# adolliou/euispice_coreg

Hardware: AMD Instinct MI355X
Metric: lag-points/sec (whole node) on 2048² grid, 60×60 CRVAL sweep; argmax-shift match (higher is better)
Workload: dtype f64; 1 GPU; headline: Carrington 'fa' 2048x2048 grid lon(200,300) lat(-20,20), 60x60 CRVAL lags arange(-30,30,1) arcsec, small 2048^2 HRIEUV-like, ref 3072^2 FSI-like, order 2, solar_r 1.004; lag_points=3600, parallelism=single GPU, no collective, resident=True, sweeps_in_flight=2, small_stored_f32=True, use_lds=True

## Files before the change

euispice_coreg_amd/csrc/host_plan.hpp:

```cpp
#pragma once
namespace {

struct ComboRange {
    long long begin = 0, end = 0;
};
ComboRange take_combo_range(coreg_handle* h) {
    ComboRange r;
    r.begin = h->opt_combo_begin;
    r.end = h->opt_combo_end;
    h->opt_combo_begin = h->opt_combo_end = 0;
    return r;
}
int check_lags(coreg_handle* h, const coreg_lags* l, LagDims* d, int64_t begin, int64_t end, ComboRange combo = ComboRange()) {
    if (!l || !l->crval1 || !l->crval2 || !l->cdelt1 || !l->cdelt2 || !l->crota)
        return fail(h, COREG_EINVAL, "lags: null array");
    if (l->n_crval1 < 1 || l->n_crval2 < 1 || l->n_cdelt1 < 1 || l->n_cdelt2 < 1 || l->n_crota < 1)
        return fail(h, COREG_EINVAL, "lags: every axis needs at least one value");
    d->n1 = l->n_crval1;
    d->n2 = l->n_crval2;
    d->n3 = l->n_cdelt1;
    d->n4 = l->n_cdelt2;
    d->n5 = l->n_crota;
    d->nc = (long long)d->n3 * d->n4 * d->n5;
    d->c0 = 0;
// ... 34 lines not shown

long long lds_window_elems(const coreg_handle* h);
SweepEnv sweep_env(coreg_handle* h) {
    SweepEnv e;
    e.sW = h->sW;
    e.sH = h->sH;
    e.gW = h->gW;
    e.gH = h->gH;
    e.border_fix = h->opt_border_fix != 0;
    e.tap_fix = h->opt_tap_fix != 0;
    e.use_lds = h->opt_use_lds != 0;
    e.h_series = h->opt_h_series != 0;
    e.tile_skip = h->opt_tile_skip != 0;
    e.lds_elems = lds_window_elems(h);
    e.tile_w = (int)h->opt_tile_w;
    e.patch_w = (int)h->opt_patch_w;
    e.shard_world = h->opt_shard_world;
    e.n_groups = h->opt_n_groups;
    e.pitch = h->opt_pitch;
    e.tabs = &h->tabs;
    e.caches = &h->wcslib;
    e.memo = &h->plan_memo;
    return e;
}

void pick_taper(const coreg_handle* h, int n_groups, int n_batches, int* tmin, int* tfrac) {
    *tmin = (int)h->opt_taper_min;
    if (h->opt_taper_frac >= 0) {
        *tfrac = (int)h->opt_taper_frac;
        return;
    }
    const double rounds = (double)n_groups * n_batches / 256.0;
    *tfrac = (rounds >= (double)h->opt_taper_rounds && n_groups >= 128 && h->opt_shard_world <= 1) ? 512 : 0;
}

template <int MODE>
int launch_precompute(coreg_handle* h, const PrecomputeArgs& a, int n_tiles, int n_groups, int n_batches) {
    EventPair* ev = next_event(h, h->ev_pre, h->ev_pre_used);
    if (!ev) return fail(h, COREG_EHIP, "hipEventCreate failed");
    int tmin, tfrac;
    pick_taper(h, n_groups, n_batches, &tmin, &tfrac);
    PrecomputeArgs b = a;
    b.prologue = h->pending_prologue;
    const bool with_prologue = b.prologue.src != nullptr;
    std::memset(&h->pending_prologue, 0, sizeof(h->pending_prologue));
    HIPCHK(hipEventRecord(ev->a, h->stream));
    if (h->ref_dtype == COREG_F32)
        hipLaunchKernelGGL((k_precompute<MODE, float>), dim3(n_tiles), dim3(256), 0, h->stream, b);
    else
        hipLaunchKernelGGL((k_precompute<MODE, double>), dim3(n_tiles), dim3(256), 0, h->stream, b);
    (void)with_prologue;
    hipLaunchKernelGGL(k_tile_list, dim3(1), dim3(1024), 0, h->stream, (const int*)a.tile_count, n_tiles, n_groups,
                       h->tile_list.as<int>(), h->tile_cum.as<int>(), h->group_first.as<int>(),
                       h->tile_info.as<long long>(), tmin, tfrac);
    ev->b_is_next_sweep = true;
    ev->next_sweep_index = h->ev_sweep_used;
    HIPCHK(hipGetLastError());
    return COREG_OK;
}

int reserve_tiles(coreg_handle* h, int n_tiles) {
    const size_t pts = (size_t)n_tiles * kTilePts + (size_t)(kPointGroups + 1) * kChunk;
    HIPCHK(h->pts.reserve(pts * sizeof(Pt)));
    HIPCHK(h->tile_count.reserve(n_tiles * sizeof(int)));
    HIPCHK(h->tile_list.reserve(n_tiles * sizeof(int)));
    HIPCHK(h->tile_cum.reserve((n_tiles + 1) * sizeof(int)));
    HIPCHK(h->group_first.reserve(2 * 1024 * sizeof(int) + 64));
    HIPCHK(h->tile_info.reserve(8 * sizeof(long long)));
    HIPCHK(h->tile_bbox.reserve((size_t)n_tiles * 4 * sizeof(double)));
    return COREG_OK;
}

int setup_precompute(coreg_handle* h, const Plan& plan, int method, PrecomputeArgs* a, int* n_tiles) {
    std::memset(a, 0, sizeof(*a));
    a->tile_w = plan.tile_w;
    a->tile_h = kTilePts / plan.tile_w;
    a->tiles_x = (h->gW + a->tile_w - 1) / a->tile_w;
    a->tiles_y = (h->gH + a->tile_h - 1) / a->tile_h;
    *n_tiles = a->tiles_x * a->tiles_y;
    RETCHK(reserve_tiles(h, *n_tiles));
    a->ref = h->ref.p;
    a->gw = h->gW;
    a->gh = h->gH;
    a->pivot_a = h->pivots.as<double>();
    a->pts = h->pts.as<Pt>();
    a->tile_count = h->tile_count.as<int>();
    a->tile_bbox = h->tile_bbox.as<double>();
    a->residus = method != COREG_METHOD_CORRELATION ? 1 : 0;
    return COREG_OK;
}

}
```

euispice_coreg_amd/csrc/host_state.hpp:

```cpp
#pragma once
namespace {

enum SrcKind {
    SRC_HOST = 0,
    SRC_PINNED = 1,
    SRC_DEVICE = 2,
    SRC_TILED = 3,
};

struct PixFmt {
    int bitpix = 0;
    bool f32 = false;
    double bscale = 1.0, bzero = 0.0;
    bool raw() const { return bitpix != 0; }
    bool scaled() const { return bscale != 1.0 || bzero != 0.0; }
    size_t elem() const { return raw() ? (size_t)(bitpix < 0 ? -bitpix : bitpix) / 8 : (f32 ? 4 : 8); }
    bool swap_only() const { return bitpix == -32 && !scaled(); }
    static PixFmt native(bool is_f32) {
        PixFmt f;
        f.f32 = is_f32;
        return f;
    }
};

// ... 5 lines not shown
    bool b_is_next_sweep = false;
    size_t next_sweep_index = 0;
};

}

struct KeptTapLists {
    DevBuf all;
};
struct TapFix {
    TapFixArgs args = {};
    int segs = 0;
    int mode = 0;
    long long count = 0;
};
struct FixLaunch {
    std::vector<BorderFixArgs> border;
    std::vector<ParityFixArgs> parity;
    TapFix tap;
    std::shared_ptr<KeptTapLists> kept;
    bool small_f32 = true;
    bool empty() const { return border.empty() && parity.empty() && tap.segs == 0; }
};

struct ContextState;
struct PixelsState;

struct coreg_handle {
    int device = 0;
    Stream stream;
    std::string err;

    std::unique_ptr<ContextState> ctx;
    std::unique_ptr<PixelsState> pix;
    ~coreg_handle();

    DevBuf small;
    int sW = 0, sH = 0;
    bool small_f32 = false;
    DevBuf ref;
    int gW = 0, gH = 0;
    int ref_dtype = -1;
    DevBuf pivots, red_sum, red_cnt;
    DevBuf t_sin_lon, t_cos_lon, t_cos_lat, t_sin_lat, t_lon_deg, t_dx;
    coreg_diffrot rot_ref = {}, rot_small = {};
    bool has_rot_ref = false, has_rot_small = false;
    CarrTables tabs;
    std::vector<double> tabs_key;
    bool tabs_uploaded = false;
    PinBuf pin_img[2];
    Event ev_img[2];
    int pin_img_next = 0;
    DevBuf pts, tile_count, tile_list, tile_cum, group_first, tile_info, tile_bbox;
    DevBuf rf_fix_slab;
    DevBuf counters;
    DevBuf lane_params, out_index, partials, out_dev, tmp_img;
    DevBuf counts;
    long long counts_n = -1;
    DevBuf up_f64, up_flag;
    DevBuf up_raw;
    DevBuf rice_blob, rice_rand, dec_img;
    PrologueArgs pending_prologue = {};
    DevBuf bbox_buf;
    Stream aux_stream;
    Stream up_stream;
    Event ev_small, ev_main;
    bool small_pending = false;
    DevBuf red_sum_up, red_cnt_up;
    int64_t opt_overlap_upload = 1;
    int64_t opt_tap_nan_filter = 2;
    int64_t opt_async_upload = 0;
    std::thread up_thread;
    std::mutex up_m;
    std::condition_variable up_cv;
    std::function<hipError_t()> up_job;
    bool up_has = false, up_stop = false, up_busy = false;
    hipError_t up_rc = hipSuccess;
    PinBuf pin_small[2];
    Event ev_pin_small[2];
    int pin_small_next = 0;
    WcslibCaches wcslib;
    DevBuf border_flags, fix_partial;
    DevBuf border_dev;
    PinBuf pin_border;
    int64_t opt_border_fix = 1;
    int64_t opt_tap_fix = 1, opt_tap_cap = 1 << 24;
    DevBuf tap_count, tap_segq, tap_list, tap_skip, tap_seg_slot, tap_seg_begin, tap_pixel, tap_xw, tap_yw;
    long long tap_last[3] = {0, 0, 0};
    int last_variant[7] = {-1, 0, 0, 0, 0, 0, 0};
    int64_t opt_shard_world = 1, opt_shard_rank = 0;
    int64_t opt_combo_begin = 0, opt_combo_end = 0;
    DevBuf sums;
    long long sums_slots = 0;
    struct PendingFinalize {
        long long slot_off, n_slots, lag_begin;
        int residus;
        RefineArgs refine;
        std::function<int(coreg_handle*)> replay_precompute;
        FixLaunch fixes;
    };
    std::function<int(coreg_handle*)> last_precompute;
    PlanMemo plan_memo;
    DevBuf rf_flags, rf_pivots, rf_list, rf_head, rf_partial;
    std::vector<PendingFinalize> pending_fin;
    DevBuf fin_outidx;
    long long pending_n_out = 0;
// ... 22 lines not shown
```

euispice_coreg_amd/csrc/host_sweep_launch.hpp:

```cpp
#pragma once
namespace {
using sweep_variant::SweepVariant;
static_assert(sweep_variant::kTranslate == MODE_TRANSLATE && sweep_variant::kHomography == MODE_HOMOGRAPHY &&
                  sweep_variant::kHomographySeries == MODE_HOMOGRAPHY_SERIES && sweep_variant::kCar == MODE_CAR &&
                  sweep_variant::kOrderRt == ORDER_RT, "sweep_variant.hpp restates the kernels' constants");

struct SweepLaunchSpec {
    int mode = MODE_TRANSLATE;
    int order = 2;
    int method = COREG_METHOD_CORRELATION;
    size_t slot_off = 0;
    int n_batches = 0, n_tiles = 0;
    long long lag_begin = 0;
    double* out_dev = nullptr;
    const LaunchU* car_inv = nullptr;
    const BorderFix* fix = nullptr;
    int pitch_sel = 0;
    long long n_slots() const { return (long long)n_batches * kBlock; }
    bool residus() const { return method != COREG_METHOD_CORRELATION; }
    int residus_kind() const { return method == COREG_METHOD_RESIDUS_MASKED ? 2 : (residus() ? 1 : 0); }
    const double* params_dev(const coreg_handle* h) const {
        return h->lane_params.as<double>() + (mode == MODE_TRANSLATE ? 2 : 9) * slot_off;
    }
    const long long* outidx_dev(const coreg_handle* h) const { return h->out_index.as<long long>() + slot_off; }
};

struct SweepKernel {
    void (*fn)(const SweepArgs);
    size_t attr_bytes[kMaxDevices];
};
template <size_t... I>
SweepKernel* sweep_kernel_table(std::index_sequence<I...>) {
    constexpr const SweepVariant* v = sweep_variant::kSweepVariants.v;
    static SweepKernel table[] = {
        {k_sweep<v[I].mode, v[I].order, std::conditional_t<v[I].f32, float, double>, v[I].round, v[I].resid, v[I].pitch>, {0}}...};
    return table;
}

int raise_dynamic_lds(coreg_handle* h, SweepKernel* k, size_t lds_bytes) {
    std::lock_guard<std::mutex> lock(g_attr_mutex);
    size_t& ab = k->attr_bytes[h->device % kMaxDevices];
    if (lds_bytes > 48 * 1024 && lds_bytes > ab) {
        HIPCHK(hipFuncSetAttribute((const void*)k->fn, hipFuncAttributeMaxDynamicSharedMemorySize, (int)lds_bytes));
        ab = lds_bytes;
    }
    return COREG_OK;
}

int launch_k_sweep(coreg_handle* h, const SweepLaunchSpec& L, const SweepArgs& a, dim3 grid, size_t lds_bytes) {
    const SweepVariant v = sweep_variant::pick_sweep_variant(L.mode, L.order, h->small_f32, L.residus(), L.pitch_sel);
    const int at = sweep_variant::sweep_variant_index(v);
    if (at < 0) return fail(h, COREG_EINVAL, "launch_sweep: no k_sweep instantiation for this mode / order / pitch");
    SweepKernel* k = sweep_kernel_table(std::make_index_sequence<sweep_variant::kNumSweepVariants>()) + at;
    EventPair* ev = next_event(h, h->ev_sweep, h->ev_sweep_used);
    if (!ev) return fail(h, COREG_EHIP, "hipEventCreate failed");
    RETCHK(raise_dynamic_lds(h, k, lds_bytes));
    HIPCHK(hipEventRecord(ev->a, h->stream));
    hipLaunchKernelGGL(k->fn, grid, dim3(kSweepThreads), lds_bytes, h->stream, a);
    HIPCHK(hipEventRecord(ev->b, h->stream));
    HIPCHK(hipGetLastError());
    const int rec[7] = {at, v.mode, v.order, v.f32 ? 1 : 0, v.round ? 1 : 0, v.resid ? 1 : 0, v.pitch};
    std::copy(rec, rec + 7, h->last_variant);
    return COREG_OK;
}

SweepArgs sweep_args(const coreg_handle* h, const SweepLaunchSpec& L, int n_groups, int group_lo, size_t lds_bytes) {
    SweepArgs a;
    a.img = h->small.p;
    a.W = h->sW;
    a.H = h->sH;
    a.pts = h->pts.as<Pt>();
    a.tile_count = h->tile_count.as<int>();
    a.tile_list = h->tile_list.as<int>();
    a.tile_cum = h->tile_cum.as<int>();
    a.group_first = h->group_first.as<int>();
    a.tile_info = h->tile_info.as<long long>();
    a.tile_bbox = h->tile_bbox.as<double>();
    a.lane_params = L.params_dev(h);
    a.n_slots = L.n_slots();
    a.n_batches = L.n_batches;
    a.n_groups = n_groups;
    a.group_lo = group_lo;
    a.partials = h->partials.as<double>();
    a.pivots = h->pivots.as<double>();
    a.use_lds = h->opt_use_lds ? 1 : 0;
    a.clean_path = h->opt_clean_path ? 1 : 0;
    a.lds_elems = (int)(lds_bytes / sizeof(double));
    a.car_inv = L.car_inv ? *L.car_inv : LaunchU{};
    a.car_inv.order_rt = L.order;
    a.car_inv.h_incr = (int)h->opt_h_incr;
    return a;
}

template <typename Args>
void fill_fix_common(Args& x, const coreg_handle* h, const SweepLaunchSpec& L) {
    x.img = h->small.p;
    x.W = h->sW;
    x.H = h->sH;
    x.ref = h->ref.p;
    x.ref_f32 = h->ref_dtype == COREG_F32 ? 1 : 0;
    x.gw = h->gW;
    x.order = L.order;
    x.round_f32 = L.mode == MODE_TRANSLATE ? 0 : 1;
    x.residus = L.residus() ? 1 : 0;
    x.pivots = h->pivots.as<double>();
    x.hom = L.params_dev(h);
    x.n_slots = L.n_slots();
}

int build_fix_launch(coreg_handle* h, const SweepLaunchSpec& L, FixLaunch* fl) {
    fl->small_f32 = h->small_f32;
    if (!L.fix || !L.fix->any()) return COREG_OK;
    static const std::vector<BorderItems::Item> no_items;
    for (const BorderItems::Item& it : L.fix->border ? L.fix->border->items : no_items) {
        if (it.flags_off >= 0) {
            ParityFixArgs p = {};
            fill_fix_common(p, h, L);
            p.flags = h->border_flags.as<unsigned char>() + it.flags_off;
            p.gh = h->gH;
            p.slot = it.slot;
            p.n_partial = 256;
            if (h->fix_partial.reserve((size_t)p.n_partial * kNumSums * sizeof(double)) != hipSuccess)
                return fail(h, COREG_EHIP, "hipMalloc failed (parity fix)");
            p.partial = h->fix_partial.as<double>();
            fl->parity.push_back(p);
        }
        if (it.n == 0) continue;
        BorderFixArgs b = {};
        fill_fix_common(b, h, L);
        b.slot = it.slot;
// ... 111 lines not shown
```

euispice_coreg_amd/csrc/kernels_prepare.hpp:

```cpp
#pragma once
namespace coreg {
template <typename T>
__global__ void __launch_bounds__(256) k_sum_finite(const T* __restrict__ v, long long n, double* part_sum,
                                                    long long* part_cnt) {
    __shared__ double ss[256];
    __shared__ long long sc[256];
    double s = 0.0;
    long long c = 0;
    for (long long i = (long long)blockIdx.x * 256 + threadIdx.x; i < n; i += (long long)gridDim.x * 256) {
        const double x = (double)v[i];
        if (isfinite(x)) {
            s += x;
            ++c;
        }
    }
    ss[threadIdx.x] = s;
    sc[threadIdx.x] = c;
    __syncthreads();
    for (int o = 128; o > 0; o >>= 1) {
        if ((int)threadIdx.x < o) {
            ss[threadIdx.x] += ss[threadIdx.x + o];
            sc[threadIdx.x] += sc[threadIdx.x + o];
        }
        __syncthreads();
// ... 262 lines not shown
                pt.pad = st;
            }
            a.pts[tbase + off + rank] = pt;
            mn0 = fmin(mn0, b0);
            mx0 = fmax(mx0, b0);
            mn1 = fmin(mn1, b1);
            mx1 = fmax(mx1, b1);
        }
        base_pos += tot;
        __syncthreads();
    }
    if (MODE != MODE_CAR && !a.residus) {
        static_assert(kChunk >= 3, "run flag + the two chunk sums live in the pads of the chunk's first three points");
        Pt* tp = a.pts + tbase;
        for (int c = threadIdx.x; c < base_pos / kChunk; c += 256) {
            double sa = tp[c * kChunk].a, saa = sa * sa;
            bool run = MODE == MODE_HOMOGRAPHY || MODE == MODE_HOMOGRAPHY_SERIES;
#pragma unroll
            for (int k = 1; k < kChunk; ++k) {
                const double v = tp[c * kChunk + k].a;
                sa += v;
                saa = fma(v, v, saa);
                run = run && tp[c * kChunk + k].b0 == tp[c * kChunk].b0 + (double)k && tp[c * kChunk + k].b1 == tp[c * kChunk].b1;
            }
            tp[c * kChunk].pad = run ? 1.0 : 0.0;
            tp[c * kChunk + 1].pad = sa;
            tp[c * kChunk + 2].pad = saa;
        }
    }
    for (int o = 32; o > 0; o >>= 1) {
        mn0 = fmin(mn0, __shfl_xor(mn0, o));
        mx0 = fmax(mx0, __shfl_xor(mx0, o));
        mn1 = fmin(mn1, __shfl_xor(mn1, o));
        mx1 = fmax(mx1, __shfl_xor(mx1, o));
    }
    if (lane == 0) {
        red[wave][0] = mn0;
        red[wave][1] = mx0;
        red[wave][2] = mn1;
        red[wave][3] = mx1;
    }
    __syncthreads();
    if (threadIdx.x == 0) {
        a.tile_count[tile] = base_pos;
        double* bb = a.tile_bbox + (size_t)tile * 4;
        bb[0] = fmin(fmin(red[0][0], red[1][0]), fmin(red[2][0], red[3][0]));
        bb[1] = fmax(fmax(red[0][1], red[1][1]), fmax(red[2][1], red[3][1]));
        bb[2] = fmin(fmin(red[0][2], red[1][2]), fmin(red[2][2], red[3][2]));
        bb[3] = fmax(fmax(red[0][3], red[1][3]), fmax(red[2][3], red[3][3]));
    }
}

constexpr int kUnitPts = kChunk * kPointGroups;
__host__ __device__ inline long long group_start(int g, long long total, int n_groups, int taper_min, int taper_frac) {
    if (taper_frac <= 0) return (long long)g * total / n_groups;
    const int g0 = n_groups - (int)((long long)n_groups * taper_frac / 1024);
    const int nt = n_groups - 1 - g0;
    if (nt <= 0) return (long long)g * total / n_groups;
    const double m = (double)taper_min / 1024.0;
    auto cum = [&](int k) -> double {
        if (k <= g0) return (double)k;
        const double j = (double)(k - g0);
        return (double)g0 + j - (1.0 - m) * j * (j - 1.0) / (2.0 * (double)nt);
    };
    if (g >= n_groups) return total;
    const long long s0 = (long long)(cum(g) / cum(n_groups) * (double)total);
    return s0 < 0 ? 0 : (s0 > total ? total : s0);
}
__global__ void __launch_bounds__(1024) k_tile_list(const int* __restrict__ tile_count, int n_tiles, int n_groups,
                                                    int* tile_list, int* tile_cum, int* group_first, long long* info,
                                                    int taper_min, int taper_frac) {
    __shared__ int wcnt[16];
    __shared__ int wunits[16];
    __shared__ long long wpts[16];
    __shared__ int s_base, s_units;
    __shared__ long long s_pts;
    const int lane = threadIdx.x & 63, wave = threadIdx.x >> 6;
    if (threadIdx.x == 0) {
        s_base = 0;
        s_units = 0;
        s_pts = 0;
    }
    __syncthreads();
    for (int t0 = 0; t0 < n_tiles; t0 += 1024) {
        const int t = t0 + threadIdx.x;
        const int c = t < n_tiles ? tile_count[t] : 0;
        const bool nz = c > 0;
        const int units = (c + kUnitPts - 1) / kUnitPts;
        const unsigned long long bal = __ballot(nz);
        const int rank = __popcll(bal & ((1ull << lane) - 1ull));
        long long pts = c;
        int uincl = units;
        for (int o = 1; o < 64; o <<= 1) {
            const int v = __shfl_up(uincl, o);
            if (lane >= o) uincl += v;
        }
        for (int o = 32; o > 0; o >>= 1) pts += __shfl_xor(pts, o);
        if (lane == 63) wunits[wave] = uincl;
        if (lane == 0) {
            wcnt[wave] = __popcll(bal);
            wpts[wave] = pts;
        }
        __syncthreads();
        int off = s_base, uoff = s_units;
        for (int w = 0; w < wave; ++w) {
            off += wcnt[w];
            uoff += wunits[w];
        }
        if (nz) {
            tile_list[off + rank] = t;
            tile_cum[off + rank] = uoff + uincl - units;
        }
        __syncthreads();
        if (threadIdx.x == 0) {
            int tot = 0, tu = 0;
            long long tp = 0;
            for (int w = 0; w < 16; ++w) {
                tot += wcnt[w];
                tu += wunits[w];
                tp += wpts[w];
            }
            s_base += tot;
            s_units += tu;
            s_pts += tp;
        }
        __syncthreads();
    }
    const int n_list = s_base, total = s_units;
    if (threadIdx.x == 0) {
        tile_cum[n_list] = total;
        info[0] = n_list;
        info[1] = s_pts;
        info[2] = total;
        info[3] = info[4] = info[5] = info[6] = 0;
    }
    __syncthreads();
    for (int g = threadIdx.x; g <= n_groups; g += 1024) {
        const long long start = group_start(g, total, n_groups, taper_min, taper_frac);
        group_first[1024 + g] = (int)start;
        int lo = 0, hi = n_list;
        while (lo < hi) {
            const int mid = (lo + hi + 1) >> 1;
            if (mid <= n_list && (long long)tile_cum[mid] <= start) lo = mid;
            else hi = mid - 1;
        }
        group_first[g] = lo;
    }
}

}
```

euispice_coreg_amd/csrc/kernels_sweep.hpp:

```cpp
#pragma once
namespace coreg {
struct SweepArgs {
    const void* img;
    int W, H;
    const Pt* pts;
    const int* tile_count;
    const int* tile_list;
    const int* tile_cum;
    const int* group_first;
    long long* tile_info;
    const double* tile_bbox;
    const double* lane_params;
    long long n_slots;
    int n_batches;
    int n_groups;
    int group_lo;
    double* partials;
    const double* pivots;
    int use_lds;
    int clean_path;
    int lds_elems;
    LaunchU car_inv;
};

struct Acc {
    int n;
    double a, b, aa, bb, ab;
};

template <int N>
struct Taps;
template <>
struct Taps<3> {
    double t[9];
    __device__ __forceinline__ void issue(unsigned a0, unsigned a1, unsigned a2) {
        asm volatile(
            "ds_read_b64 %0, %9\n\tds_read_b64 %1, %9 offset:8\n\tds_read_b64 %2, %9 offset:16\n\t"
            "ds_read_b64 %3, %10\n\tds_read_b64 %4, %10 offset:8\n\tds_read_b64 %5, %10 offset:16\n\t"
            "ds_read_b64 %6, %11\n\tds_read_b64 %7, %11 offset:8\n\tds_read_b64 %8, %11 offset:16"
            : "=&v"(t[0]), "=&v"(t[1]), "=&v"(t[2]), "=&v"(t[3]), "=&v"(t[4]), "=&v"(t[5]), "=&v"(t[6]), "=&v"(t[7]),
              "=&v"(t[8])
            : "v"(a0), "v"(a1), "v"(a2));
    }
    __device__ __forceinline__ void wait_after(double& w0, double& w1, double& w2, double& w3, double& w4, double& w5) {
        asm volatile("s_waitcnt lgkmcnt(0)"
                     : "+v"(t[0]), "+v"(t[1]), "+v"(t[2]), "+v"(t[3]), "+v"(t[4]), "+v"(t[5]), "+v"(t[6]), "+v"(t[7]),
                       "+v"(t[8]), "+v"(w0), "+v"(w1), "+v"(w2), "+v"(w3), "+v"(w4), "+v"(w5));
    }
    __device__ __forceinline__ void issue_before(unsigned a0, unsigned a1, unsigned a2, double& fx, double& fy) {
        asm volatile(
            "ds_read_b64 %0, %11\n\tds_read_b64 %1, %11 offset:8\n\tds_read_b64 %2, %11 offset:16\n\t"
            "ds_read_b64 %3, %12\n\tds_read_b64 %4, %12 offset:8\n\tds_read_b64 %5, %12 offset:16\n\t"
            "ds_read_b64 %6, %13\n\tds_read_b64 %7, %13 offset:8\n\tds_read_b64 %8, %13 offset:16"
            : "=&v"(t[0]), "=&v"(t[1]), "=&v"(t[2]), "=&v"(t[3]), "=&v"(t[4]), "=&v"(t[5]), "=&v"(t[6]), "=&v"(t[7]),
              "=&v"(t[8]), "+v"(fx), "+v"(fy)
            : "v"(a0), "v"(a1), "v"(a2));
    }
    __device__ __forceinline__ void wait() {
        asm volatile("s_waitcnt lgkmcnt(0)"
                     : "+v"(t[0]), "+v"(t[1]), "+v"(t[2]), "+v"(t[3]), "+v"(t[4]), "+v"(t[5]), "+v"(t[6]), "+v"(t[7]),
                       "+v"(t[8]));
    }
    template <int P>
    __device__ __forceinline__ void issue_before_imm(unsigned a0, double& fx, double& fy) {
// ... 312 lines not shown
        } else if (isfinite(v)) {
            acc.n += 1;
            acc.a += av;
            acc.b += bm;
            acc.aa = fma(av, av, acc.aa);
            acc.bb = fma(bm, bm, acc.bb);
            acc.ab = fma(av, bm, acc.ab);
        }
    }
}

#ifndef COREG_PT_SCALAR
#define COREG_PT_SCALAR 2
#endif
#ifndef COREG_PT_ANCHOR
#define COREG_PT_ANCHOR 1
#endif
typedef unsigned SPt __attribute__((ext_vector_type(8)));
__device__ __forceinline__ SPt spt_load(const Pt* __restrict__ p, double& anchor) {
    SPt r;
#if defined(__HIP_DEVICE_COMPILE__)
#if COREG_PT_ANCHOR
    asm volatile("s_load_dwordx8 %0, %2, 0x0" : "=s"(r), "+v"(anchor) : "s"(p));
#else
    asm volatile("s_load_dwordx8 %0, %1, 0x0" : "=s"(r) : "s"(p));
#endif
#else
    r = (SPt)(0u);
    (void)p;
    (void)anchor;
#endif
    return r;
}
__device__ __forceinline__ void spt_wait(SPt& r) {
#if defined(__HIP_DEVICE_COMPILE__)
    asm volatile("s_waitcnt lgkmcnt(0)" : "+s"(r));
#endif
}
__device__ __forceinline__ double spt_f64(const SPt& r, int i) {
    const unsigned long long u = ((unsigned long long)r[2 * i + 1] << 32) | (unsigned long long)r[2 * i];
    return __builtin_bit_cast(double, u);
}
__device__ __forceinline__ void load_pt_uniform(const Pt* __restrict__ p, Pt& out) {
#if defined(__HIP_DEVICE_COMPILE__) && COREG_PT_SCALAR
    typedef const __attribute__((address_space(4))) double* ConstF64;
    ConstF64 q = (ConstF64)(const double*)p;
    out.b0 = q[0];
    out.b1 = q[1];
    out.a = q[2];
    out.pad = q[3];
#else
    out = *p;
#endif
}

template <int MODE, int ORDER, typename TS, bool LDS, bool ROUND, bool RESID, bool INTERIOR = false, int PITCH = 0,
          bool CLEAN = false>
__device__ __forceinline__ void tile_points(Acc& acc, unsigned win, const TS* __restrict__ img, int pitch,
                                            int ox, int oy, int W, int H, double px0, double py0, double pxw,
                                            double pyw, const H9& hm, const LaunchU& cu, const Pt* __restrict__ pts, int p_begin, int p_end,
                                            double pivot_b, int pg) {
    const double wmax = (double)(W - 1), hmax = (double)(H - 1);
    const int n_full = p_end / kChunk;
#if defined(__HIP_DEVICE_COMPILE__) && COREG_PT_SCALAR == 2
    constexpr bool kIncr = INTERIOR && LDS && ORDER == 2 && !RESID &&
                           (MODE == MODE_HOMOGRAPHY || MODE == MODE_HOMOGRAPHY_SERIES);
    if constexpr (kIncr) {
        if (cu.h_incr) {
            H9 hv = hm;
            hv.h[0] = fma(pxw, hm.h[6], hm.h[0]);
            hv.h[1] = fma(pxw, hm.h[7], hm.h[1]);
            hv.h[2] = MODE == MODE_HOMOGRAPHY_SERIES ? hm.h[2] + pxw : fma(pxw, hm.h[8], hm.h[2]);
            hv.h[3] = fma(pyw, hm.h[6], hm.h[3]);
            hv.h[4] = fma(pyw, hm.h[7], hm.h[4]);
            hv.h[5] = MODE == MODE_HOMOGRAPHY_SERIES ? hm.h[5] + pyw : fma(pyw, hm.h[8], hm.h[5]);
            int c = p_begin / kChunk + pg;
            if (c < n_full) {
                double& anchor = hv.h[7];
                SPt cur = spt_load(pts + c * kChunk, anchor);
                spt_wait(cur);
                for (; c < n_full; c += kPointGroups) {
                    const Pt* __restrict__ q = pts + c * kChunk;
                    const bool run = cur[7] != 0u;
                    double xn = 0.0, yn = 0.0, ww = 0.0;
#pragma unroll
                    for (int k = 0; k < kChunk; ++k) {
                        SPt nxt = spt_load(k + 1 < kChunk ? q + k + 1 : q + kPointGroups * kChunk, anchor);
                        const double x = spt_f64(cur, 0), y = spt_f64(cur, 1);
                        if (k == 0 || !run) {
                            xn = fma(hv.h[0], x, fma(hv.h[1], y, hv.h[2]));
                            yn = fma(hv.h[3], x, fma(hv.h[4], y, hv.h[5]));
                            ww = MODE == MODE_HOMOGRAPHY_SERIES ? fma(hv.h[6], x, hv.h[7] * y)
                                                                : fma(hv.h[6], x, fma(hv.h[7], y, hv.h[8]));
                        } else {
                            xn += hv.h[0];
                            yn += hv.h[3];
                            ww += hv.h[6];
                        }
                        double ux, uy;
                        if (MODE == MODE_HOMOGRAPHY_SERIES) {
                            const double qq = fma(ww, ww, -ww);
                            ux = fma(xn, qq, xn);
                            uy = fma(yn, qq, yn);
                        } else {
                            double r = __builtin_amdgcn_rcp(ww);
                            r = fma(r, fma(-ww, r, 1.0), r);
// ... 75 lines not shown
            load_pt_uniform(pts + p, pt);
            point_lag<MODE, ORDER, TS, LDS, ROUND, RESID, INTERIOR, PITCH>(acc, win, img, pitch, ox, oy, W, H, wmax, hmax,
                                                                           px0, py0, pxw, pyw, hm, cu, pt.b0, pt.b1, pt.a,
                                                                           pt.pad, pivot_b);
        }
    }
}

template <int MODE, int ORDER, typename TS, bool ROUND, bool RESID, int PITCH = 0>
__global__ void __launch_bounds__(kSweepThreads) k_sweep(const SweepArgs a) {
    extern __shared__ __align__(16) unsigned char lds_raw[];
    double* lds = (double*)lds_raw;
    constexpr int kWaves = kSweepThreads / 64;
    constexpr int kLagWaves = kBlock / 64;
    __shared__ double wred2[2][kLagWaves][4];
    __shared__ int wdirty[2][kWaves];
    constexpr bool kCleanPath = MODE != MODE_CAR && !RESID && ORDER != ORDER_RT && !(ROUND && sizeof(TS) == 8);
    int visit = 0;
    int n_vis = 0, n_vis_lds = 0, n_vis_int = 0, n_vis_clean = 0;

    const int b = blockIdx.x;
    const int slot8 = b & 7;
    const int q = b >> 3;
    const int batch = q % a.n_batches;
    const int group = a.group_lo + (q / a.n_batches) * 8 + slot8;

    const int lane = threadIdx.x & 63, wave = threadIdx.x >> 6;
    const int pg = __builtin_amdgcn_readfirstlane(wave % kPointGroups);
    const int lw = __builtin_amdgcn_readfirstlane(wave / kPointGroups);
    const int ls = 64 * lw + lane;
    const long long slot = (long long)batch * kBlock + ls;

    double px0 = 0.0, py0 = 0.0;
    H9 hm;
#pragma unroll
    for (int k = 0; k < 9; ++k) hm.h[k] = 0.0;
    if (MODE == MODE_TRANSLATE) {
        px0 = a.lane_params[slot];
        py0 = a.lane_params[a.n_slots + slot];
    } else {
#pragma unroll
        for (int k = 0; k < 9; ++k) hm.h[k] = a.lane_params[(long long)k * a.n_slots + slot];
    }

    const bool pad_lane = MODE == MODE_TRANSLATE ? (px0 != px0) : (hm.h[8] != hm.h[8]);

    Acc acc = {0, 0.0, 0.0, 0.0, 0.0, 0.0};

    const TS* __restrict__ img = (const TS*)a.img;
    const int W = a.W, H = a.H;
    const double inf = __builtin_inf();
    const int u_lo = a.group_first[1024 + group];
    const int u_hi = a.group_first[1024 + group + 1];
    const int n_list = (int)a.tile_info[0];
    const double pivot_b = a.pivots[1];
#if defined(__HIP_DEVICE_COMPILE__)
    const unsigned win = (unsigned)(uintptr_t)(__attribute__((address_space(3))) unsigned char*)lds_raw;
#else
    const unsigned win = 0;
#endif

    for (int tl = a.group_first[group]; tl < n_list && u_lo < u_hi; ++tl) {
        const int ubase = a.tile_cum[tl];
        if (ubase >= u_hi) break;
        const int tile = a.tile_list[tl];
        const int cnt = a.tile_count[tile];
        const int p_begin = max(u_lo - ubase, 0) * kUnitPts;
        const int p_end = min((u_hi - ubase) * kUnitPts, cnt);
        if (p_begin >= p_end) continue;
        const double* bb = a.tile_bbox + (size_t)tile * 4;
        const double bx0 = bb[0], bx1 = bb[1], by0 = bb[2], by1 = bb[3];

        double mnx, mxx, mny, mxy;
        if (MODE == MODE_TRANSLATE) {
            mnx = bx0 + px0;
            mxx = bx1 + px0;
            mny = by0 + py0;
            mxy = by1 + py0;
        } else {
            mnx = inf; mxx = -inf; mny = inf; mxy = -inf;
#pragma unroll
            for (int c = 0; c < 4; ++c) {
                double cx, cy;
                apply_map<MODE>(hm, a.car_inv, (c & 1) ? bx1 : bx0, (c & 2) ? by1 : by0, cx, cy);
                mnx = fmin(mnx, cx);
                mxx = fmax(mxx, cx);
                mny = fmin(mny, cy);
                mxy = fmax(mxy, cy);
            }
            if (MODE == MODE_CAR) {
                const double margin = car_tile_margin(a.car_inv.box_c, fmax(fabs(by0), fabs(by1)) + a.car_inv.pole_sep);
                mnx -= margin;
                mxx += margin;
                mny -= margin;
                mxy += margin;
            }
        }
        for (int o = 32; o > 0; o >>= 1) {
            mnx = fmin(mnx, __shfl_xor(mnx, o));
            mxx = fmax(mxx, __shfl_xor(mxx, o));
            mny = fmin(mny, __shfl_xor(mny, o));
            mxy = fmax(mxy, __shfl_xor(mxy, o));
        }
        double(*wred)[4] = wred2[visit & 1];
        int* wdirt = wdirty[visit & 1];
        ++visit;
        if (lane == 0 && pg == 0) {
            wred[lw][0] = mnx;
            wred[lw][1] = mxx;
            wred[lw][2] = mny;
            wred[lw][3] = mxy;
        }
        __syncthreads();
        mnx = fmin(fmin(wred[0][0], wred[1][0]), fmin(wred[2][0], wred[3][0]));
        mxx = fmax(fmax(wred[0][1], wred[1][1]), fmax(wred[2][1], wred[3][1]));
        mny = fmin(fmin(wred[0][2], wred[1][2]), fmin(wred[2][2], wred[3][2]));
        mxy = fmax(fmax(wred[0][3], wred[1][3]), fmax(wred[2][3], wred[3][3]));
        if (!(mxx >= 0.0) || !(mnx <= (double)(W - 1)) || !(mxy >= 0.0) || !(mny <= (double)(H - 1))) continue;
        constexpr double kClear = 1e-9;
        const bool interior = (mnx >= kClear) & (mxx <= (double)(W - 1) - kClear) & (mny >= kClear) &
                              (mxy <= (double)(H - 1) - kClear);
        constexpr bool kWide = ORDER == ORDER_RT || ORDER > 2;
        const int ord = ORDER == ORDER_RT ? a.car_inv.order_rt : ORDER;
        const int ap_lo = kWide ? ord / 2 + 1 : 1;
        const int ap_hi = kWide ? ord - ord / 2 + 1 : 2;
        const int ox = max((int)floor(fmax(mnx, 0.0)) - ap_lo, kWide ? -ap_lo : -1);
        const int oy = max((int)floor(fmax(mny, 0.0)) - ap_lo, kWide ? -ap_lo : -1);
        const int ex = min((int)floor(fmin(mxx, (double)(W - 1))) + ap_hi, kWide ? W - 1 + ap_hi : W);
        const int ey = min((int)floor(fmin(mxy, (double)(H - 1))) + ap_hi, kWide ? H - 1 + ap_hi : H);
        const int ww = ex - ox + 1, wh = ey - oy + 1;
        int pitch = PITCH > 0 ? PITCH : (ww | 1);
        if (PITCH == 0) {
            const int r = pitch & 31;
            const int up = r < 5 ? 5 - r : ((r > 11 && r < 21) ? 21 - r : (r > 27 ? 37 - r : 0));
            if ((long long)(pitch + up) * wh <= (long long)a.lds_elems) pitch += up;
        }
        const long long need = (long long)pitch * wh;
        const bool in_lds = a.use_lds && (need <= (long long)a.lds_elems) && (PITCH == 0 || ww <= PITCH);

        const Pt* __restrict__ pts = a.pts + (size_t)tile * kTilePts;

        bool swept = false;
        ++n_vis;
        {
          if (in_lds) {
            swept = true;
            ++n_vis_lds;
#ifndef COREG_STAGE_ROWS
#define COREG_STAGE_ROWS 8
#endif
#ifndef COREG_STAGE_COLS
#define COREG_STAGE_COLS 1
#endif
            constexpr int kStage = COREG_STAGE_ROWS, kCols = COREG_STAGE_COLS;
            const double scale = ORDER == 2 ? 0.25 : 1.0;
            const int wave_u = __builtin_amdgcn_readfirstlane(wave);
            double poison = 0.0;
            for (int r0 = wave_u; r0 < wh; r0 += kWaves * kStage) {
                for (int c0 = 0; c0 < ww; c0 += 64 * kCols) {
                    int gx[kCols];
#pragma unroll
                    for (int j = 0; j < kCols; ++j) {
                        const int c = c0 + 64 * j + lane;
                        gx[j] = kWide ? mirror_far(ox + min(c, ww - 1), W) : mirror_idx(ox + min(c, ww - 1), W);
                    }
                    TS v[kStage][kCols];
#pragma unroll
                    for (int k = 0; k < kStage; ++k) {
                        const int r = min(r0 + k * kWaves, wh - 1);
                        const int gy = kWide ? mirror_far(oy + r, H) : mirror_idx(oy + r, H);
                        const TS* __restrict__ row = img + (size_t)gy * W;
#pragma unroll
                        for (int j = 0; j < kCols; ++j) v[k][j] = row[gx[j]];
                    }
#pragma unroll
                    for (int j = 0; j < kCols; ++j) {
                        const int c = c0 + 64 * j + lane;
                        if (c < ww) {
#pragma unroll
                            for (int k = 0; k < kStage; ++k) {
                                const int r = r0 + k * kWaves;
                                if (r < wh) {
                                    const double e = (ROUND ? (double)v[k][j] : (double)v[k][j] - pivot_b) * scale;
                                    lds[r * pitch + c] = e;
                                    if (kCleanPath) poison = fma(e, 0.0, poison);
                                }
                            }
                        }
                    }
                }
            }
            if (kCleanPath && interior) {
                const int dirty = __ballot(poison != poison) != 0ull;
                if (lane == 0) wdirt[wave] = dirty;
            }
            __syncthreads();
            bool done = false;
            if constexpr (ORDER != ORDER_RT) {
                if (interior) {
                    done = true;
                    bool clean = false;
                    if constexpr (kCleanPath) clean = a.clean_path && __ballot(wdirt[lane % kWaves] != 0) == 0ull;
                    ++n_vis_int;
                    n_vis_clean += clean ? 1 : 0;
                    if (!pad_lane) {
                        const double offx = (ORDER == 2 ? 0.5 : 0.0) - (double)(ORDER / 2 + ox);
                        const double offy = (ORDER == 2 ? 0.5 : 0.0) - (double)(ORDER / 2 + oy);
                        const double pxw = MODE == MODE_TRANSLATE ? px0 + offx : offx;
                        const double pyw = MODE == MODE_TRANSLATE ? py0 + offy : offy;
                        if (kCleanPath && clean) {
                            tile_points<MODE, ORDER, TS, true, ROUND, RESID, true, PITCH, kCleanPath>(
                                acc, win, img, pitch, ox, oy, W, H, px0, py0, pxw, pyw, hm, a.car_inv, pts, p_begin, p_end,
                                pivot_b, pg);
                        } else {
                            tile_points<MODE, ORDER, TS, true, ROUND, RESID, true, PITCH>(acc, win, img, pitch, ox, oy, W, H,
                                                                                          px0, py0, pxw, pyw, hm, a.car_inv,
                                                                                          pts, p_begin, p_end, pivot_b, pg);
                        }
                    }
                }
            }
            if (!done) {
                const double offx = ORDER == 2 ? 0.5 - (double)(1 + ox) : (ORDER == 3 ? -(double)(1 + ox) : 0.0);
                const double offy = ORDER == 2 ? 0.5 - (double)(1 + oy) : (ORDER == 3 ? -(double)(1 + oy) : 0.0);
                tile_points<MODE, ORDER, TS, true, ROUND, RESID, false, PITCH>(acc, win, img, pitch, ox, oy, W, H, px0, py0,
                                                                               offx, offy, hm, a.car_inv, pts, p_begin,
                                                                               p_end, pivot_b, pg);
            }
          }
        }
        if (!swept) {
            tile_points<MODE, ORDER, TS, false, ROUND, RESID>(acc, win, img, 0, 0, 0, W, H, px0, py0, 0.0, 0.0, hm, a.car_inv, pts,
                                                              p_begin, p_end, pivot_b, pg);
        }
    }

    if (threadIdx.x == 0) {
        atomicAdd((unsigned long long*)a.tile_info + 3, (unsigned long long)n_vis);
        atomicAdd((unsigned long long*)a.tile_info + 4, (unsigned long long)n_vis_lds);
        atomicAdd((unsigned long long*)a.tile_info + 5, (unsigned long long)n_vis_int);
        atomicAdd((unsigned long long*)a.tile_info + 6, (unsigned long long)n_vis_clean);
    }
    __syncthreads();
    if (pg > 0) {
        double* st = lds + ((size_t)(pg - 1) * kNumSums) * kBlock + ls;
        st[0] = (double)acc.n;
        st[kBlock] = acc.a;
        st[2 * kBlock] = acc.b;
        st[3 * kBlock] = acc.aa;
        st[4 * kBlock] = acc.bb;
        st[5 * kBlock] = acc.ab;
    }
    __syncthreads();
    if (pg == 0) {
        double sn = (double)acc.n, sa = acc.a, sb = acc.b, saa = acc.aa, sbb = acc.bb, sab = acc.ab;
        for (int g = 0; g < kPointGroups - 1; ++g) {
            const double* st = lds + ((size_t)g * kNumSums) * kBlock + ls;
            sn += st[0];
            sa += st[kBlock];
            sb += st[2 * kBlock];
            saa += st[3 * kBlock];
            sbb += st[4 * kBlock];
            sab += st[5 * kBlock];
        }
        double* out = a.partials + (size_t)(group - a.group_lo) * kNumSums * a.n_slots + slot;
        out[0] = sn;
        out[a.n_slots] = sa;
        out[2 * a.n_slots] = sb;
        out[3 * a.n_slots] = saa;
        out[4 * a.n_slots] = sbb;
        out[5 * a.n_slots] = sab;
    }
}

}
```

Baseline: 1.208 million lag-points/s.

## Pack per-visit tile records, prefetch next visit, hoist lag bounding box

Builds a 64-byte VisitRec per listed tile (cumulative units, tile id, count, bbox) in k_tile_list. The sweep kernel loads each record through scalar constant-address loads, prefetches the next one and parks it in a VGPR via writelane. For translate mode it computes the lag bounding box once per block, so the per-visit wave shuffle reduction and one barrier per visit go away. It also folds the order-2 staging subtract-and-scale into a single FMA. The intent is to cut dependent global loads and syncs per tile visit, at the cost of a looser (union-over-lanes) window bound and more staged rows.

```diff
diff --git a/euispice_coreg_amd/csrc/host_plan.hpp b/euispice_coreg_amd/csrc/host_plan.hpp
--- a/euispice_coreg_amd/csrc/host_plan.hpp
+++ b/euispice_coreg_amd/csrc/host_plan.hpp
@@ -110,7 +110,8 @@
     (void)with_prologue;
     hipLaunchKernelGGL(k_tile_list, dim3(1), dim3(1024), 0, h->stream, (const int*)a.tile_count, n_tiles, n_groups,
                        h->tile_list.as<int>(), h->tile_cum.as<int>(), h->group_first.as<int>(),
-                       h->tile_info.as<long long>(), tmin, tfrac);
+                       h->tile_info.as<long long>(), tmin, tfrac, (const double*)a.tile_bbox,
+                       h->visit_rec.as<VisitRec>());
     ev->b_is_next_sweep = true;
     ev->next_sweep_index = h->ev_sweep_used;
     HIPCHK(hipGetLastError());
@@ -126,6 +127,7 @@
     HIPCHK(h->group_first.reserve(2 * 1024 * sizeof(int) + 64));
     HIPCHK(h->tile_info.reserve(8 * sizeof(long long)));
     HIPCHK(h->tile_bbox.reserve((size_t)n_tiles * 4 * sizeof(double)));
+    HIPCHK(h->visit_rec.reserve(((size_t)n_tiles + 1) * sizeof(VisitRec)));
     return COREG_OK;
 }
 
diff --git a/euispice_coreg_amd/csrc/host_state.hpp b/euispice_coreg_amd/csrc/host_state.hpp
--- a/euispice_coreg_amd/csrc/host_state.hpp
+++ b/euispice_coreg_amd/csrc/host_state.hpp
@@ -81,6 +81,7 @@
     Event ev_img[2];
     int pin_img_next = 0;
     DevBuf pts, tile_count, tile_list, tile_cum, group_first, tile_info, tile_bbox;
+    DevBuf visit_rec;
     DevBuf rf_fix_slab;
     DevBuf counters;
     DevBuf lane_params, out_index, partials, out_dev, tmp_img;
diff --git a/euispice_coreg_amd/csrc/host_sweep_launch.hpp b/euispice_coreg_amd/csrc/host_sweep_launch.hpp
--- a/euispice_coreg_amd/csrc/host_sweep_launch.hpp
+++ b/euispice_coreg_amd/csrc/host_sweep_launch.hpp
@@ -76,6 +76,7 @@
     a.group_first = h->group_first.as<int>();
     a.tile_info = h->tile_info.as<long long>();
     a.tile_bbox = h->tile_bbox.as<double>();
+    a.visit_rec = h->visit_rec.as<VisitRec>();
     a.lane_params = L.params_dev(h);
     a.n_slots = L.n_slots();
     a.n_batches = L.n_batches;
diff --git a/euispice_coreg_amd/csrc/kernels_prepare.hpp b/euispice_coreg_amd/csrc/kernels_prepare.hpp
--- a/euispice_coreg_amd/csrc/kernels_prepare.hpp
+++ b/euispice_coreg_amd/csrc/kernels_prepare.hpp
@@ -338,6 +338,12 @@
 }
 
 constexpr int kUnitPts = kChunk * kPointGroups;
+struct alignas(64) VisitRec {
+    int tile_cum, tile, count, pad;
+    double bbox[4];
+    double fill[2];
+};
+static_assert(sizeof(VisitRec) == 64, "one record per 64-byte line");
 __host__ __device__ inline long long group_start(int g, long long total, int n_groups, int taper_min, int taper_frac) {
     if (taper_frac <= 0) return (long long)g * total / n_groups;
     const int g0 = n_groups - (int)((long long)n_groups * taper_frac / 1024);
@@ -355,7 +361,8 @@
 }
 __global__ void __launch_bounds__(1024) k_tile_list(const int* __restrict__ tile_count, int n_tiles, int n_groups,
                                                     int* tile_list, int* tile_cum, int* group_first, long long* info,
-                                                    int taper_min, int taper_frac) {
+                                                    int taper_min, int taper_frac,
+                                                    const double* __restrict__ tile_bbox, VisitRec* visit_rec) {
     __shared__ int wcnt[16];
     __shared__ int wunits[16];
     __shared__ long long wpts[16];
@@ -396,6 +403,15 @@
         if (nz) {
             tile_list[off + rank] = t;
             tile_cum[off + rank] = uoff + uincl - units;
+            VisitRec r;
+            r.tile_cum = uoff + uincl - units;
+            r.tile = t;
+            r.count = c;
+            r.pad = 0;
+#pragma unroll
+            for (int k = 0; k < 4; ++k) r.bbox[k] = tile_bbox[(size_t)t * 4 + k];
+            r.fill[0] = r.fill[1] = 0.0;
+            visit_rec[off + rank] = r;
         }
         __syncthreads();
         if (threadIdx.x == 0) {
@@ -415,6 +431,9 @@
     const int n_list = s_base, total = s_units;
     if (threadIdx.x == 0) {
         tile_cum[n_list] = total;
+        VisitRec r = {};
+        r.tile_cum = total;
+        visit_rec[n_list] = r;
         info[0] = n_list;
         info[1] = s_pts;
         info[2] = total;
diff --git a/euispice_coreg_amd/csrc/kernels_sweep.hpp b/euispice_coreg_amd/csrc/kernels_sweep.hpp
--- a/euispice_coreg_amd/csrc/kernels_sweep.hpp
+++ b/euispice_coreg_amd/csrc/kernels_sweep.hpp
@@ -10,6 +10,7 @@
     const int* group_first;
     long long* tile_info;
     const double* tile_bbox;
+    const VisitRec* visit_rec;
     const double* lane_params;
     long long n_slots;
     int n_batches;
@@ -428,6 +429,83 @@
 #else
     out = *p;
 #endif
+}
+
+#ifndef COREG_VISIT_LAGBOX
+#define COREG_VISIT_LAGBOX 1
+#endif
+#ifndef COREG_VISIT_FMA
+#define COREG_VISIT_FMA 1
+#endif
+struct Visit {
+    int ubase, tile, cnt;
+    double bx0, bx1, by0, by1;
+};
+__device__ __forceinline__ void load_visit_uniform(const VisitRec* __restrict__ p, Visit& out) {
+#if defined(__HIP_DEVICE_COMPILE__)
+    typedef const __attribute__((address_space(4))) int* ConstI32;
+    typedef const __attribute__((address_space(4))) double* ConstF64;
+    ConstI32 qi = (ConstI32)(const int*)p;
+    ConstF64 qd = (ConstF64)(const double*)p;
+    out.ubase = qi[0];
+    out.tile = qi[1];
+    out.cnt = qi[2];
+    out.bx0 = qd[2];
+    out.bx1 = qd[3];
+    out.by0 = qd[4];
+    out.by1 = qd[5];
+#else
+    out.ubase = p->tile_cum;
+    out.tile = p->tile;
+    out.cnt = p->count;
+    out.bx0 = p->bbox[0];
+    out.bx1 = p->bbox[1];
+    out.by0 = p->bbox[2];
+    out.by1 = p->bbox[3];
+#endif
+}
+template <int LANE>
+__device__ __forceinline__ void write_lane(unsigned& w, unsigned x) {
+#if defined(__HIP_DEVICE_COMPILE__)
+    asm("v_writelane_b32 %0, %1, %2" : "+v"(w) : "s"(x), "n"(LANE));
+#else
+    (void)w;
+    (void)x;
+#endif
+}
+__device__ __forceinline__ unsigned park_visit(const Visit& v, unsigned park) {
+    const unsigned long long b[4] = {__builtin_bit_cast(unsigned long long, v.bx0), __builtin_bit_cast(unsigned long long, v.bx1),
+                                     __builtin_bit_cast(unsigned long long, v.by0), __builtin_bit_cast(unsigned long long, v.by1)};
+    unsigned w = park;
+    write_lane<0>(w, (unsigned)v.ubase);
+    write_lane<1>(w, (unsigned)v.tile);
+    write_lane<2>(w, (unsigned)v.cnt);
+    write_lane<3>(w, (unsigned)b[0]);
+    write_lane<4>(w, (unsigned)(b[0] >> 32));
+    write_lane<5>(w, (unsigned)b[1]);
+    write_lane<6>(w, (unsigned)(b[1] >> 32));
+    write_lane<7>(w, (unsigned)b[2]);
+    write_lane<8>(w, (unsigned)(b[2] >> 32));
+    write_lane<9>(w, (unsigned)b[3]);
+    write_lane<10>(w, (unsigned)(b[3] >> 32));
+    return w;
+}
+__device__ __forceinline__ void unpark_visit(unsigned park, Visit& v) {
+    const int w = (int)park;
+    v.ubase = __builtin_amdgcn_readlane(w, 0);
+    v.tile = __builtin_amdgcn_readlane(w, 1);
+    v.cnt = __builtin_amdgcn_readlane(w, 2);
+    double b[4];
+#pragma unroll
+    for (int k = 0; k < 4; ++k) {
+        const unsigned lo = (unsigned)__builtin_amdgcn_readlane(w, 3 + 2 * k);
+        const unsigned hi = (unsigned)__builtin_amdgcn_readlane(w, 4 + 2 * k);
+        b[k] = __builtin_bit_cast(double, ((unsigned long long)hi << 32) | (unsigned long long)lo);
+    }
+    v.bx0 = b[0];
+    v.bx1 = b[1];
+    v.by0 = b[2];
+    v.by1 = b[3];
 }
 
 template <int MODE, int ORDER, typename TS, bool LDS, bool ROUND, bool RESID, bool INTERIOR = false, int PITCH = 0,
@@ -609,7 +687,6 @@
     const double inf = __builtin_inf();
     const int u_lo = a.group_first[1024 + group];
     const int u_hi = a.group_first[1024 + group + 1];
-    const int n_list = (int)a.tile_info[0];
     const double pivot_b = a.pivots[1];
 #if defined(__HIP_DEVICE_COMPILE__)
     const unsigned win = (unsigned)(uintptr_t)(__attribute__((address_space(3))) unsigned char*)lds_raw;
@@ -617,19 +694,61 @@
     const unsigned win = 0;
 #endif
 
-    for (int tl = a.group_first[group]; tl < n_list && u_lo < u_hi; ++tl) {
-        const int ubase = a.tile_cum[tl];
+    constexpr bool kLagBox = MODE == MODE_TRANSLATE && COREG_VISIT_LAGBOX;
+    double lx0 = 0.0, lx1 = 0.0, ly0 = 0.0, ly1 = 0.0;
+    if constexpr (kLagBox) {
+        lx0 = lx1 = px0;
+        ly0 = ly1 = py0;
+        for (int o = 32; o > 0; o >>= 1) {
+            lx0 = fmin(lx0, __shfl_xor(lx0, o));
+            lx1 = fmax(lx1, __shfl_xor(lx1, o));
+            ly0 = fmin(ly0, __shfl_xor(ly0, o));
+            ly1 = fmax(ly1, __shfl_xor(ly1, o));
+        }
+        if (lane == 0 && pg == 0) {
+            wred2[0][lw][0] = lx0;
+            wred2[0][lw][1] = lx1;
+            wred2[0][lw][2] = ly0;
+            wred2[0][lw][3] = ly1;
+        }
+        __syncthreads();
+        lx0 = fmin(fmin(wred2[0][0][0], wred2[0][1][0]), fmin(wred2[0][2][0], wred2[0][3][0]));
+        lx1 = fmax(fmax(wred2[0][0][1], wred2[0][1][1]), fmax(wred2[0][2][1], wred2[0][3][1]));
+        ly0 = fmin(fmin(wred2[0][0][2], wred2[0][1][2]), fmin(wred2[0][2][2], wred2[0][3][2]));
+        ly1 = fmax(fmax(wred2[0][0][3], wred2[0][1][3]), fmax(wred2[0][2][3], wred2[0][3][3]));
+    }
+
+    int tl = a.group_first[group];
+    unsigned park = 0;
+    {
+        Visit first;
+        load_visit_uniform(a.visit_rec + tl, first);
+        park = park_visit(first, park);
+    }
+    for (; u_lo < u_hi; ++tl) {
+        Visit cur;
+        unpark_visit(park, cur);
+        const int ubase = cur.ubase;
         if (ubase >= u_hi) break;
-        const int tile = a.tile_list[tl];
-        const int cnt = a.tile_count[tile];
+        Visit nxt;
+        load_visit_uniform(a.visit_rec + tl + 1, nxt);
+        const int tile = cur.tile;
+        const int cnt = cur.cnt;
         const int p_begin = max(u_lo - ubase, 0) * kUnitPts;
         const int p_end = min((u_hi - ubase) * kUnitPts, cnt);
-        if (p_begin >= p_end) continue;
-        const double* bb = a.tile_bbox + (size_t)tile * 4;
-        const double bx0 = bb[0], bx1 = bb[1], by0 = bb[2], by1 = bb[3];
+        if (p_begin >= p_end) {
+            park = park_visit(nxt, park);
+            continue;
+        }
+        const double bx0 = cur.bx0, bx1 = cur.bx1, by0 = cur.by0, by1 = cur.by1;
 
         double mnx, mxx, mny, mxy;
-        if (MODE == MODE_TRANSLATE) {
+        if constexpr (kLagBox) {
+            mnx = bx0 + lx0;
+            mxx = bx1 + lx1;
+            mny = by0 + ly0;
+            mxy = by1 + ly1;
+        } else if (MODE == MODE_TRANSLATE) {
             mnx = bx0 + px0;
             mxx = bx1 + px0;
             mny = by0 + py0;
@@ -653,27 +772,33 @@
                 mxy += margin;
             }
         }
-        for (int o = 32; o > 0; o >>= 1) {
-            mnx = fmin(mnx, __shfl_xor(mnx, o));
-            mxx = fmax(mxx, __shfl_xor(mxx, o));
-            mny = fmin(mny, __shfl_xor(mny, o));
-            mxy = fmax(mxy, __shfl_xor(mxy, o));
-        }
-        double(*wred)[4] = wred2[visit & 1];
         int* wdirt = wdirty[visit & 1];
+        if constexpr (!kLagBox) {
+            for (int o = 32; o > 0; o >>= 1) {
+                mnx = fmin(mnx, __shfl_xor(mnx, o));
+                mxx = fmax(mxx, __shfl_xor(mxx, o));
+                mny = fmin(mny, __shfl_xor(mny, o));
+                mxy = fmax(mxy, __shfl_xor(mxy, o));
+            }
+            double(*wred)[4] = wred2[visit & 1];
+            if (lane == 0 && pg == 0) {
+                wred[lw][0] = mnx;
+                wred[lw][1] = mxx;
+                wred[lw][2] = mny;
+                wred[lw][3] = mxy;
+            }
+            __syncthreads();
+            mnx = fmin(fmin(wred[0][0], wred[1][0]), fmin(wred[2][0], wred[3][0]));
+            mxx = fmax(fmax(wred[0][1], wred[1][1]), fmax(wred[2][1], wred[3][1]));
+            mny = fmin(fmin(wred[0][2], wred[1][2]), fmin(wred[2][2], wred[3][2]));
+            mxy = fmax(fmax(wred[0][3], wred[1][3]), fmax(wred[2][3], wred[3][3]));
+        }
         ++visit;
-        if (lane == 0 && pg == 0) {
-            wred[lw][0] = mnx;
-            wred[lw][1] = mxx;
-            wred[lw][2] = mny;
-            wred[lw][3] = mxy;
-        }
-        __syncthreads();
-        mnx = fmin(fmin(wred[0][0], wred[1][0]), fmin(wred[2][0], wred[3][0]));
-        mxx = fmax(fmax(wred[0][1], wred[1][1]), fmax(wred[2][1], wred[3][1]));
-        mny = fmin(fmin(wred[0][2], wred[1][2]), fmin(wred[2][2], wred[3][2]));
-        mxy = fmax(fmax(wred[0][3], wred[1][3]), fmax(wred[2][3], wred[3][3]));
-        if (!(mxx >= 0.0) || !(mnx <= (double)(W - 1)) || !(mxy >= 0.0) || !(mny <= (double)(H - 1))) continue;
+        if (!(mxx >= 0.0) || !(mnx <= (double)(W - 1)) || !(mxy >= 0.0) || !(mny <= (double)(H - 1))) {
+            park = park_visit(nxt, park);
+            continue;
+        }
+        if constexpr (kLagBox) __syncthreads();
         constexpr double kClear = 1e-9;
         const bool interior = (mnx >= kClear) & (mxx <= (double)(W - 1) - kClear) & (mny >= kClear) &
                               (mxy <= (double)(H - 1) - kClear);
@@ -711,6 +836,8 @@
 #endif
             constexpr int kStage = COREG_STAGE_ROWS, kCols = COREG_STAGE_COLS;
             const double scale = ORDER == 2 ? 0.25 : 1.0;
+            constexpr bool kFmaStage = ORDER == 2 && !ROUND && COREG_VISIT_FMA;
+            const double npivot4 = -0.25 * pivot_b;
             const int wave_u = __builtin_amdgcn_readfirstlane(wave);
             double poison = 0.0;
             for (int r0 = wave_u; r0 < wh; r0 += kWaves * kStage) {
@@ -738,7 +865,8 @@
                             for (int k = 0; k < kStage; ++k) {
                                 const int r = r0 + k * kWaves;
                                 if (r < wh) {
-                                    const double e = (ROUND ? (double)v[k][j] : (double)v[k][j] - pivot_b) * scale;
+                                    const double e = (kFmaStage ? fma((double)v[k][j], 0.25, npivot4)
+                                                                : (ROUND ? (double)v[k][j] : (double)v[k][j] - pivot_b) * scale);
                                     lds[r * pitch + c] = e;
                                     if (kCleanPath) poison = fma(e, 0.0, poison);
                                 }
@@ -747,6 +875,7 @@
                     }
                 }
             }
+            park = park_visit(nxt, park);
             if (kCleanPath && interior) {
                 const int dirty = __ballot(poison != poison) != 0ull;
                 if (lane == 0) wdirt[wave] = dirty;
@@ -787,6 +916,7 @@
           }
         }
         if (!swept) {
+            park = park_visit(nxt, park);
             tile_points<MODE, ORDER, TS, false, ROUND, RESID>(acc, win, img, 0, 0, 0, W, H, px0, py0, 0.0, 0.0, hm, a.car_inv, pts,
                                                               p_begin, p_end, pivot_b, pg);
         }
```

After: 1.235 million lag-points/s, median of 6. 2.2% higher.
